# LanaSina/evolutionary_illusion_generator

Hardware: AMD Instinct MI355X
Metric: genome fitness evals/sec at 256x256, pop=256 (higher is better)
Workload: dtype f32; 1 GPU; neat_configs/circles.txt colour pop=256, 256x256, PredNet 3,48,96,192, 21 steps, LK + rotation-symmetry score; global_pop=256, genomes_per_gpu=256, device_batch=256, structure=Circles

## Files before the change

evolutionary_illusion_generator_amd/csrc/conv_wino4.h:

```cpp
#pragma once
#include "wino_launch.h"

namespace eig {

constexpr int W4_UPOS = 256;
constexpr int W4_U_FLOATS = W4_NPOS * W4_UPOS;
constexpr int W4_NUS = 3, W4_NPS = 3;
constexpr int w4_row(bool tall) { return tall ? 28 : 40; }
constexpr int w4_ps(bool tall) { return tall ? 1024 : 768; }
constexpr int w4_pslot(bool tall) { return W4_KC * w4_ps(tall); }
constexpr int w4_p(bool tall, int k) { return tall ? k * w4_pslot(true) : (k < 2 ? k * w4_pslot(false) : 2 * w4_pslot(false) + 3 * W4_U_FLOATS); }
constexpr int w4_u(bool tall, int k) { return tall ? 3 * w4_pslot(true) + k * W4_U_FLOATS : 2 * w4_pslot(false) + k * W4_U_FLOATS; }
constexpr int w4_x(bool tall) { return tall ? w4_u(true, 0) : w4_u(false, 1); }
constexpr int W4_X_FLOATS = W4_WAVES * 2 * 4 * 64 * 4;
constexpr int wino4_lds_bytes() { return (w4_x(false) + W4_X_FLOATS) * 4; }
static_assert((w4_u(true, 2) + W4_U_FLOATS) * 4 == wino4_lds_bytes() && (w4_p(false, 2) + w4_pslot(false)) * 4 <= wino4_lds_bytes(), "LDS maps");
#ifndef EIG_W4_DEEPU
#define EIG_W4_DEEPU 1
#endif
#ifndef EIG_W4_DIAG
#define EIG_W4_DIAG 0
#endif

__device__ __forceinline__ void w4_in1d(float d0, float d1, float d2, float d3, float d4, float d5, float* T)
{
    T[0] = fmaf(4.0f, d0, fmaf(-5.0f, d2, d4));
    const float p = fmaf(-4.0f, d2, d4), q = fmaf(-4.0f, d1, d3);
    T[1] = p + q; T[2] = p - q;
    const float r = d4 - d2, s = d3 - d1;
    T[3] = fmaf(2.0f, s, r); T[4] = fmaf(-2.0f, s, r);
    T[5] = fmaf(4.0f, d1, fmaf(-5.0f, d3, d5));
}
template <int XI> __device__ __forceinline__ float w4_row(const float* d)
{
    if constexpr (XI == 0) return fmaf(4.0f, d[0], fmaf(-5.0f, d[1], d[2]));
    else if constexpr (XI == 5) return fmaf(4.0f, d[0], fmaf(-5.0f, d[1], d[2]));
    else {
        if constexpr (XI == 1) return fmaf(-4.0f, d[1], d[3]) + fmaf(-4.0f, d[0], d[2]);
        else if constexpr (XI == 2) return fmaf(-4.0f, d[1], d[3]) - fmaf(-4.0f, d[0], d[2]);
        else if constexpr (XI == 3) return fmaf(2.0f, d[2] - d[0], d[3] - d[1]);
        else return fmaf(-2.0f, d[2] - d[0], d[3] - d[1]);
    }
}
constexpr int w4_nrows(int xi) { return (xi == 0 || xi == 5) ? 3 : 4; }
constexpr int w4_rowidx(int xi, int k) { return xi == 0 ? 2 * k : xi == 5 ? 2 * k + 1 : k + 1; }
constexpr int w4_uprow(int i) { return (i + 1) >> 1; }

template <typename V4> __device__ __forceinline__ void w4_out1d(const V4& m0, const V4& m1, const V4& m2, const V4& m3, const V4& m4, const V4& m5, V4* Y)
{
    const V4 s = m1 + m2, d = m1 - m2, u = m3 + m4, w = m3 - m4;
    Y[0] = (m0 + s) + u;
    for (int e = 0; e < 4; ++e) { Y[1][e] = fmaf(2.0f, w[e], d[e]); Y[2][e] = fmaf(4.0f, u[e], s[e]); Y[3][e] = fmaf(8.0f, w[e], d[e]) + m5[e]; }
}

template <int NI, int EPI, bool TALL = false, bool HALF = false, bool PACK = false, bool NSPLIT = false>
__global__ void __launch_bounds__((HALF && !NSPLIT) ? W4_THREADS / 2 : W4_THREADS, 3) wino4_kernel(const ConvArgs a)
{
    static_assert(!NSPLIT || (HALF && NI == 4 && EPI != EPI_CONVA), "N-split: a half block, 64-column N-blocks, ConvLSTM / ConvP");
    constexpr int NIW = NSPLIT ? 2 : NI;
    constexpr bool DEEPU = HALF && EIG_W4_DEEPU;
    static_assert(!(TALL && HALF), "half blocks exist in the wide shape only");
    static_assert(!PACK || (HALF && EPI != EPI_CONVA), "packed tiles: a half block, ConvLSTM / ConvP");
    constexpr bool TGEO = TALL || PACK;
    static_assert(EPI == EPI_LSTM || EPI == EPI_CONVA || EPI == EPI_CONVP, "conv_wino4.h: ConvLSTM, ConvA, ConvP");
    static_assert(EPI != EPI_LSTM || NI == 4, "ConvLSTM: the four N-tiles are the four gates");
    static_assert(NI == 3 || NI == 4, "N-blocks of 48 or 64 columns");
    constexpr int U4 = wino4_u_floats(NI);
    constexpr int KC = W4_KC, PS = w4_ps(TGEO), W4_ROW = w4_row(TGEO);
    constexpr int W4_P0 = w4_p(TGEO, 0), W4_P1 = w4_p(TGEO, 1), W4_P2 = w4_p(TGEO, 2), W4_U0 = w4_u(TGEO, 0), W4_U1 = w4_u(TGEO, 1), W4_U2 = w4_u(TGEO, 2);
    constexpr int PK_ROWS = 18, PK_CX = 7, PK_IMG = PK_ROWS * PK_CX;
    constexpr bool WALK = !TALL && !HALF;
    constexpr int RGH = TALL ? 16 : 8;
    extern __shared__ __attribute__((aligned(16))) float lds[];
    unsigned long long tq_entry = EIG_TIMING ? __builtin_readcyclecounter() : 0;
    float* const Pb = lds;
    float* const Ub = lds;
    float* const xb = lds + w4_x(TGEO);
    const int wv_o = __builtin_amdgcn_readfirstlane((int)threadIdx.x >> 6);
    const int rg_o = HALF ? 0 : wv_o & 1, xi_o = (HALF && !NSPLIT) ? wv_o : wv_o >> 1;
    const int ng_o = NSPLIT ? wv_o & 1 : 0;
    constexpr int NWAVES = (HALF && !NSPLIT) ? W4_WAVES / 2 : W4_WAVES;
    constexpr int UPW = 36 / NWAVES;
    auto lane_id = [&]() __attribute__((always_inline)) { int l = (int)__builtin_amdgcn_mbcnt_hi(~0u, __builtin_amdgcn_mbcnt_lo(~0u, 0u)); asm volatile("" : "+v"(l)); return l; };

    const int tiles = a.tilesX * a.tilesY;
    const bool pk5 = PACK && a.tilesX == 5;
    const int ntile = PACK ? a.B + (pk5 ? (a.B + 3) >> 2 : 0) : a.B * tiles;
    const int xcd = blockIdx.x & 7, xi_ = blockIdx.x >> 3;
    auto dv = [&](int x, int d, unsigned m) __attribute__((always_inline)) { return m ? (int)__umulhi((unsigned)x, m) : x / d; };
    const int q0 = dv(xi_, a.nparts, a.mg[0]);
    const int part = xi_ - q0 * a.nparts;
    const int tlin = a.tile_map ? xcd * ((ntile + 7) >> 3) + q0 : q0 * 8 + xcd;
    if (tlin >= ntile) return;
    const int nwalk = WALK ? a.nwalk : 1, nb0 = part * nwalk;
    const bool pk_edge_o = pk5 && tlin >= a.B;
    const int eb = PACK ? (pk_edge_o ? 4 * (tlin - a.B) : tlin) : dv(tlin, tiles, a.mg[1]);
    const int t_ = PACK ? 0 : tlin - eb * tiles;
    const int tyi = dv(t_, a.tilesX, a.mg[2]), txi = t_ - tyi * a.tilesX;
    const int y0 = PACK ? 0 : tyi * (TALL ? 32 : (HALF ? 8 : 16)), x0 = PACK ? 0 : txi * (TALL ? 16 : 32);
    const int HW = a.H * a.W;

    const bool up_fused = !PACK && EPI == EPI_LSTM && a.up_src != nullptr;
    const int nkb0 = a.src[0].C / KC;
    const int nkbu = up_fused ? (a.up_C / KC) : 0;
    const bool has1 = a.nsrc > 1;
    const int nkb_o = nkb0 + nkbu + (has1 ? (a.src[1].C / KC) : 0);
    const int up_lo_o = nkb0, up_hi_o = nkb0 + nkbu;
#define EIG4_WAITCNT(imm) do { __builtin_amdgcn_s_waitcnt(imm); asm volatile("" ::: "memory"); } while (0)
#define EIG4_BARRIER() do { asm volatile("" ::: "memory"); __builtin_amdgcn_s_barrier(); asm volatile("" ::: "memory"); } while (0)
#define EIG4_LDS_BARRIER() do { EIG4_WAITCNT(0xC07F); EIG4_BARRIER(); } while (0)
#define EIG4_IS_UP(kb) ((kb) >= up_lo && (kb) < up_hi)

    typedef float f32x2 __attribute__((ext_vector_type(2)));
    constexpr unsigned W4_POSB = 4 * 16 * NI * 4;
    auto walk_body = [&](const int it) __attribute__((always_inline)) {
    const int nblk = nb0 + it;
    int zs = 0;
    asm volatile("" : "+s"(zs));
    const int wv = wv_o + zs, rg = rg_o + zs, xi = xi_o + zs, ng = ng_o + zs, nkb = nkb_o + zs, up_lo = up_lo_o + zs, up_hi = up_hi_o + zs;
    const int pch = HALF ? wv >> 1 : wv / 3, ppart = HALF ? wv & 1 : wv - pch * 3;
    const bool has_plane = !(NSPLIT && !PACK) || wv_o < 8;
    const int eb_i = eb + zs, y0_i = y0 + zs, x0_i = x0 + zs;
    const bool pk_edge = (pk_edge_o ? 1 : 0) + zs != 0;
    const unsigned long long sb0 = (unsigned long long)(a.src[0].ptr + (size_t)eb_i * a.src[0].Ct * HW);
    const unsigned long long sb1 = has1 ? (unsigned long long)(a.src[1].ptr + (size_t)eb_i * a.src[1].Ct * HW) : sb0;
    const int ist0 = a.src[0].Ct * HW * 4, ist1 = has1 ? a.src[1].Ct * HW * 4 : ist0;
    const int sz0 = a.src[0].C * HW * 4 + (PACK ? 3 * ist0 : 0), sz1 = has1 ? a.src[1].C * HW * 4 + (PACK ? 3 * ist1 : 0) : sz0;
    const int Hh = a.H >> 1, Wh = a.W >> 1, HWh = Hh * Wh;
    const unsigned long long sbu = up_fused ? (unsigned long long)(a.up_src + (size_t)eb_i * a.up_C * HWh) : sb0;
    const int szu = up_fused ? a.up_C * HWh * 4 : sz0;
    const int lane = lane_id();
    const int q = lane >> 4, col = lane & 15;
    constexpr int CPR = TALL ? 7 : 10, CREAL = TALL ? 6 : 10, NCHK = TALL ? 34 * 7 : (HALF ? 100 : 180), UROWS = TALL ? 18 : (HALF ? 6 : 10), UCHK = TALL ? 4 : 6;
    auto plane_offsets = [&](int part, int& ro, int& uo) __attribute__((always_inline)) {
        const int c = lane + 64 * part;
        const int row = c / CPR, cx = c - row * CPR;
        const int gy = y0_i - 1 + row, gx = x0_i - 4 + 4 * cx;
        ro = (c < NCHK && cx < CREAL && gy >= 0 && gy < a.H && gx >= 0 && gx < a.W) ? (gy * a.W + gx) * 4 : -1;
        const int hy = (y0_i >> 1) - 1 + row, hx = (x0_i >> 1) - 4 + 4 * cx;
        uo = (row < UROWS && cx < UCHK && hy >= 0 && hy < Hh && hx >= 0 && hx < Wh) ? (hy * Wh + hx) * 4 : -1;
    };
    int pk_ro[3] = {-1, -1, -1};
    unsigned pk_mul[3] = {0u, 0u, 0u};
    const int pk_n = (wv_o < 4 ? 2 : 1) + (NSPLIT ? 0 : 1);
    if constexpr (PACK) {
#pragma unroll
        for (int k = 0; k < 3; ++k) {
            const int c = lane + 64 * ((wv_o + NWAVES * k) & 3);
            const int p = c >= PK_IMG ? 1 : 0, c1 = c - PK_IMG * p;
            const int row = c1 / PK_CX, slot = c1 - row * PK_CX;
            const int b = slot >= 3 ? (slot >= 6 ? 2 : 1) : 0;
            const int irel = pk_edge ? 2 * p + b : 0, cx = pk_edge ? 4 + slot - 3 * b : slot;
            const int gy = row - 1, gx = 4 * cx - 4;
            const bool ok = (pk_edge ? (c < 2 * PK_IMG && b < 2) : c < PK_IMG) && eb_i + irel < a.B && gy >= 0 && gy < a.H && gx >= 0 && gx < a.W;
            pk_ro[k] = ok ? (gy * a.W + gx) * 4 : -1;
            pk_mul[k] = ok ? (unsigned)irel : 0u;
        }
    }
    int roff, uoff, roff2 = -1, uoff2 = -1;
    plane_offsets(ppart, roff, uoff);
    const bool two_parts = (TALL && wv_o < 4) || (HALF && !PACK && !NSPLIT && wv_o < 2);
    if (TALL) plane_offsets(3, roff2, uoff2);
    if (HALF) { roff2 = roff; uoff2 = uoff; }
    const int ch2 = HALF ? 3 : wv, part2 = HALF ? ppart : 3;
    auto dma_plane_at = [&](int jj, int slot_off) __attribute__((always_inline)) {
        const int j = jj < nkb ? jj : nkb - 1;
        const bool up = EIG4_IS_UP(j);
        const bool s1 = j >= up_hi;
        const unsigned long long mu = 0ull - (unsigned long long)up, m1 = 0ull - (unsigned long long)s1;
        const unsigned long long u = sb0 + ((sb1 - sb0) & m1) + ((sbu - sb0) & mu);
        const unsigned lo = __builtin_amdgcn_readfirstlane((unsigned)u), hi = __builtin_amdgcn_readfirstlane((unsigned)(u >> 32));
        const int sz = sz0 + ((sz1 - sz0) & (int)m1) + ((szu - sz0) & (int)mu);
        const __amdgpu_buffer_rsrc_t rs = __builtin_amdgcn_make_buffer_rsrc((void*)(((unsigned long long)hi << 32) | lo), 0, __builtin_amdgcn_readfirstlane(sz), 0x00020000);
        const int base = (up_lo & (int)mu) + (up_hi & (int)m1), hw = HW + ((HWh - HW) & (int)mu);
        if constexpr (PACK) {
            const unsigned ist = (unsigned)(ist0 + ((ist1 - ist0) & (int)m1));
#pragma unroll
            for (int k = 0; k < 3; ++k) {
                if (k >= pk_n) break;
                const int idx = wv_o + NWAVES * k;
                const unsigned coffk = (unsigned)((j - base) * KC + (idx >> 2)) * (unsigned)(hw * 4);
                __builtin_amdgcn_raw_ptr_buffer_load_lds(rs, (__attribute__((address_space(3))) void*)(Pb + slot_off + (idx >> 2) * PS + (idx & 3) * 256), 16,
                                                         (int)__builtin_elementwise_add_sat((unsigned)pk_ro[k] + pk_mul[k] * ist, coffk), 0, 0, 0);
            }
            return;
        }
        if (!has_plane) return;
        const unsigned coff = (unsigned)((j - base) * KC + pch) * (unsigned)(hw * 4);
        __builtin_amdgcn_raw_ptr_buffer_load_lds(rs, (__attribute__((address_space(3))) void*)(Pb + slot_off + pch * PS + ppart * 256), 16,
                                                 (int)__builtin_elementwise_add_sat((unsigned)roff + (((unsigned)uoff - (unsigned)roff) & (unsigned)mu), coff), 0, 0, 0);
        if (two_parts) {
            const unsigned coff2 = (unsigned)((j - base) * KC + ch2) * (unsigned)(hw * 4);
            __builtin_amdgcn_raw_ptr_buffer_load_lds(rs, (__attribute__((address_space(3))) void*)(Pb + slot_off + ch2 * PS + part2 * 256), 16,
                                                     (int)__builtin_elementwise_add_sat((unsigned)roff2 + (((unsigned)uoff2 - (unsigned)roff2) & (unsigned)mu), coff2), 0, 0, 0);
        }
    };
    auto wait_u = [&]() __attribute__((always_inline)) {
        const int npl = PACK ? pk_n : (two_parts ? 2 : (has_plane ? 1 : 0));
        switch (npl + (DEEPU ? UPW : 0)) {
            case 0: EIG4_WAITCNT(0x0F70); break;
            case 1: EIG4_WAITCNT(0x0F71); break;
            case 2: EIG4_WAITCNT(0x0F72); break;
            case 3: EIG4_WAITCNT(0x0F73); break;
            case 4: EIG4_WAITCNT(0x0F74); break;
            case 5: EIG4_WAITCNT(0x0F75); break;
            case 6: EIG4_WAITCNT(0x0F76); break;
            case 7: EIG4_WAITCNT(0x0F77); break;
            case 8: EIG4_WAITCNT(0x0F78); break;
            default: EIG4_WAITCNT(0x0F79); break;
        }
    };
    const int uvo = (NI == 4 || lane < 48) ? lane * 16 : -1;
    auto prologue_a = [&](int nb) __attribute__((always_inline)) {
        const __amdgpu_buffer_rsrc_t rs = __builtin_amdgcn_make_buffer_rsrc((void*)(a.wpk + (size_t)nb * nkb * U4), 0, (nkb + 1) * U4 * 4, 0x00020000);
#pragma unroll
        for (int i = 0; i < UPW; ++i)
            __builtin_amdgcn_raw_ptr_buffer_load_lds(rs, (__attribute__((address_space(3))) void*)(Ub + W4_U0 + (UPW * wv + i) * W4_UPOS), 16, uvo, (int)((unsigned)(UPW * wv + i) * W4_POSB), 0, 0);
        dma_plane_at(0, W4_P0);
        dma_plane_at(1, W4_P1);
    };
    auto prologue_b = [&](int nb) __attribute__((always_inline)) {
        const __amdgpu_buffer_rsrc_t rs = __builtin_amdgcn_make_buffer_rsrc((void*)(a.wpk + (size_t)nb * nkb * U4), 0, (nkb + 1) * U4 * 4, 0x00020000);
#pragma unroll
        for (int i = 0; i < UPW; ++i)
            __builtin_amdgcn_raw_ptr_buffer_load_lds(rs, (__attribute__((address_space(3))) void*)(Ub + W4_U1 + (UPW * wv + i) * W4_UPOS), 16, uvo,
                                                     (int)((unsigned)U4 * 4 + (unsigned)(UPW * wv + i) * W4_POSB), 0, 0);
        dma_plane_at(2, W4_P2);
    };

    const int pk_ir = pk_edge ? col >> 2 : 0, pk_ty = pk_edge ? col & 3 : col >> 2;
    const int t_ty = PACK ? 0 : (TALL ? col >> 2 : col >> 3), t_tx = PACK ? (pk_edge ? 3 * (pk_ir & 1) : col & 3) : (TALL ? col & 3 : col & 7);
    const int pk_row = PACK ? PK_ROWS * (pk_ir >> 1) + 4 * pk_ty : 0;
    const float* const pbase_n = Pb + q * PS + (RGH * rg + 4 * t_ty + pk_row) * W4_ROW + 4 * t_tx;
    const float* const pbase_u = Pb + q * PS + ((RGH / 2) * rg + 2 * t_ty) * W4_ROW + 2 * t_tx + 3;
    const int b_off = xi * 6 * W4_UPOS + (q * 16 + col) * NI + 2 * ng;

    unsigned long long tq_setup = tq_entry;
    if (it == 0) {
        if (EIG_TIMING) tq_setup = __builtin_readcyclecounter();
        prologue_a(nb0);
        EIG4_WAITCNT(0x0F70);
    }
    const __amdgpu_buffer_rsrc_t rsw = __builtin_amdgcn_make_buffer_rsrc((void*)(a.wpk + (size_t)nblk * nkb * U4), 0, (nkb + 1) * U4 * 4, 0x00020000);
    unsigned u_so = (unsigned)(UPW * wv) * W4_POSB + 2u * (unsigned)U4 * 4u;
    auto dma_u = [&](int slot_off) __attribute__((always_inline)) {
#pragma unroll
        for (int i = 0; i < UPW; ++i)
            __builtin_amdgcn_raw_ptr_buffer_load_lds(rsw, (__attribute__((address_space(3))) void*)(Ub + slot_off + (UPW * wv + i) * W4_UPOS), 16, uvo,
                                                     (int)(u_so + (unsigned)i * W4_POSB), 0, 0);
        u_so += (unsigned)U4 * 4;
    };
    f32x4 acc[6][NIW];
#pragma unroll
    for (int p = 0; p < 6; ++p)
#pragma unroll
        for (int ni = 0; ni < NIW; ++ni) acc[p][ni] = (f32x4){0.f, 0.f, 0.f, 0.f};
    EIG4_BARRIER();
    prologue_b(nblk);
    const unsigned long long tq_k0 = EIG_TIMING ? __builtin_readcyclecounter() : 0;
    unsigned long long tq_k1 = 0, tq_x = 0, tq_y = 0;
    auto timeline = [&]() __attribute__((always_inline)) {
        if (EIG_TIMING && a.dbg && lane_id() == 0) {
            unsigned hwid, xcc;
            asm volatile("s_getreg_b32 %0, hwreg(HW_REG_HW_ID)" : "=s"(hwid));
            asm volatile("s_getreg_b32 %0, hwreg(HW_REG_XCC_ID)" : "=s"(xcc));
            unsigned long long* dd = a.dbg + (((size_t)blockIdx.x * nwalk + it) * NWAVES + wv) * 8;
            const unsigned long long tq_end = __builtin_readcyclecounter();
            dd[0] = tq_entry; dd[1] = tq_setup; dd[2] = tq_k0; dd[3] = tq_k1; dd[4] = tq_x; dd[5] = tq_y; dd[6] = tq_end;
            dd[7] = (unsigned long long)hwid | ((unsigned long long)xcc << 32);
            tq_entry = tq_end;
        }
    };

    auto kloops = [&](auto role_tag) __attribute__((always_inline)) {
        constexpr int XI = decltype(role_tag)::value;
        float v[6];
        float bq[NIW];
        int uo0 = W4_U0, uo1 = W4_U1, uo2 = W4_U2;
        int po0 = W4_P0, po1 = W4_P1, po2 = W4_P2;
        int pj = 0, psz = 0, pbound = 0;
        unsigned pcoff = 0, plo = 0, phi = 0, phw4 = 0, pist = 0;
        bool pup = false;
        auto plane_source = [&](int j) __attribute__((always_inline)) {
            const bool up = EIG4_IS_UP(j);
            const bool s1 = j >= up_hi;
            const unsigned long long mu = 0ull - (unsigned long long)up, m1 = 0ull - (unsigned long long)s1;
            const unsigned long long u = sb0 + ((sb1 - sb0) & m1) + ((sbu - sb0) & mu);
            plo = __builtin_amdgcn_readfirstlane((unsigned)u); phi = __builtin_amdgcn_readfirstlane((unsigned)(u >> 32));
            psz = __builtin_amdgcn_readfirstlane(sz0 + ((sz1 - sz0) & (int)m1) + ((szu - sz0) & (int)mu));
            const int base = (up_lo & (int)mu) + (up_hi & (int)m1);
            phw4 = (unsigned)((HW + ((HWh - HW) & (int)mu)) * 4);
            pcoff = (unsigned)((j - base) * KC + (PACK ? 0 : pch)) * phw4;
            if constexpr (PACK) pist = (unsigned)(ist0 + ((ist1 - ist0) & (int)m1));
            pup = up; pj = j;
            pbound = j < up_lo ? up_lo : (j < up_hi ? up_hi : nkb);
        };
        auto dma_plane = [&]() __attribute__((always_inline)) {
            const unsigned o = (unsigned)roff + (((unsigned)uoff - (unsigned)roff) & (0u - (unsigned)pup));
            const __amdgpu_buffer_rsrc_t prs = __builtin_amdgcn_make_buffer_rsrc((void*)(((unsigned long long)phi << 32) | plo), 0, psz, 0x00020000);
            if constexpr (PACK) {
#pragma unroll
                for (int k = 0; k < 3; ++k) {
                    if (k >= pk_n) break;
                    const int idx = wv + NWAVES * k;
                    __builtin_amdgcn_raw_ptr_buffer_load_lds(prs, (__attribute__((address_space(3))) void*)(Pb + po0 + (idx >> 2) * PS + (idx & 3) * 256), 16,
                                                             (int)__builtin_elementwise_add_sat((unsigned)pk_ro[k] + pk_mul[k] * pist, pcoff + (unsigned)(idx >> 2) * phw4), 0, 0, 0);
                }
            } else if (has_plane) {
            __builtin_amdgcn_raw_ptr_buffer_load_lds(prs, (__attribute__((address_space(3))) void*)(Pb + po0 + pch * PS + ppart * 256), 16,
                                                     (int)__builtin_elementwise_add_sat(o, pcoff), 0, 0, 0);
            }
            if (two_parts) {
                const unsigned o2 = (unsigned)roff2 + (((unsigned)uoff2 - (unsigned)roff2) & (0u - (unsigned)pup));
                __builtin_amdgcn_raw_ptr_buffer_load_lds(prs, (__attribute__((address_space(3))) void*)(Pb + po0 + ch2 * PS + part2 * 256), 16,
                                                         (int)__builtin_elementwise_add_sat(o2, pcoff + (unsigned)(ch2 - pch) * phw4), 0, 0, 0);
            }
            ++pj; pcoff += KC * phw4;
            if (__builtin_expect(pj == pbound, 0)) {
                if (pbound < nkb) plane_source(pj);
                else { --pj; pcoff -= KC * phw4; }
            }
        };
        plane_source(3 < nkb ? 3 : nkb - 1);
        float pr[2][6];
        float t[6];
        int rso = 0;
        bool rup = false;
        auto read_rows = [&](int ph) __attribute__((always_inline)) {
            if (EIG_W4_DIAG & 4) return;
            constexpr bool END = XI == 0 || XI == 5;
#pragma unroll
            for (int j = 0; j < 2; ++j) {
                const int k = ph == 0 ? (END ? 1 + j : 1 + 2 * j) : (END ? 0 : 2 * j);
                if (ph == 1 && END && j == 1) continue;
                if (rup) {
                    const float* const pl = pbase_u + rso + w4_uprow(w4_rowidx(XI, k)) * W4_ROW;
                    const float s0 = pl[0], s1_ = pl[1], s2 = pl[2], s3 = pl[3];
                    pr[j][0] = s0; pr[j][1] = s1_; pr[j][2] = s1_; pr[j][3] = s2; pr[j][4] = s2; pr[j][5] = s3;
                } else {
                    const float* const pl = pbase_n + rso + w4_rowidx(XI, k) * W4_ROW;
                    typedef const volatile __attribute__((address_space(3))) f32x2* lds_f32x2;
                    const f32x2 c0 = *(lds_f32x2)(pl + 2), c2 = *(lds_f32x2)(pl + 8);
                    const f32x4 c1 = *reinterpret_cast<const f32x4*>(pl + 4);
                    pr[j][0] = c0[1]; pr[j][1] = c1[0]; pr[j][2] = c1[1]; pr[j][3] = c1[2]; pr[j][4] = c1[3]; pr[j][5] = c2[0];
                }
            }
        };
        auto rows_begin = [&](int slot_off, bool up) __attribute__((always_inline)) {
            rso = slot_off; rup = up;
            read_rows(0);
        };
        auto rows_mid = [&]() __attribute__((always_inline)) {
            if (!(EIG_W4_DIAG & 4)) {
#pragma unroll
                for (int c = 0; c < 6; ++c) {
                    if constexpr (XI == 0 || XI == 5) t[c] = fmaf(-5.0f, pr[0][c], pr[1][c]);
                    else if constexpr (XI == 1 || XI == 2) t[c] = fmaf(-4.0f, pr[0][c], pr[1][c]);
                    else t[c] = pr[1][c] - pr[0][c];
                }
            }
            read_rows(1);
        };
        auto rows_end = [&]() __attribute__((always_inline)) {
            if (EIG_W4_DIAG & 4) return;
#pragma unroll
            for (int c = 0; c < 6; ++c) {
                if constexpr (XI == 0 || XI == 5) t[c] = fmaf(4.0f, pr[0][c], t[c]);
                else if constexpr (XI == 1) t[c] = t[c] + fmaf(-4.0f, pr[0][c], pr[1][c]);
                else if constexpr (XI == 2) t[c] = t[c] - fmaf(-4.0f, pr[0][c], pr[1][c]);
                else if constexpr (XI == 3) t[c] = fmaf(2.0f, pr[1][c] - pr[0][c], t[c]);
                else t[c] = fmaf(-2.0f, pr[1][c] - pr[0][c], t[c]);
            }
        };
        auto build_cols = [&]() __attribute__((always_inline)) {
            if (EIG_W4_DIAG & 4) { for (int c = 0; c < 6; ++c) v[c] = 1.0f; return; }
            w4_in1d(t[0], t[1], t[2], t[3], t[4], t[5], v);
        };
        auto read_b = [&](int slot_off, int nu, float* dst) __attribute__((always_inline)) {
            const float* const bsrc = Ub + slot_off + b_off + nu * W4_UPOS;
            if constexpr (NSPLIT) {
                const f32x2 b2 = *reinterpret_cast<const f32x2*>(bsrc);
                dst[0] = b2[0]; dst[1] = b2[1];
            } else if constexpr (NI == 4) {
                const f32x4 b4 = *reinterpret_cast<const f32x4*>(bsrc);
                dst[0] = b4[0]; dst[1] = b4[1]; dst[2] = b4[2]; dst[3] = b4[3];
            } else {
#pragma unroll
                for (int ni = 0; ni < NI; ++ni) dst[ni] = bsrc[ni];
            }
        };
        float bv[2][NIW];
        auto khead_mfma = [&]() __attribute__((always_inline)) {
            __builtin_amdgcn_sched_barrier(0);
            acc[0][0] = __builtin_amdgcn_mfma_f32_16x16x4f32(v[0], bq[0], acc[0][0], 0, 0, 0);
            __builtin_amdgcn_sched_barrier(0);
            read_b(uo0, 1, bv[1]);
#pragma unroll
            for (int ni = 1; ni < NIW; ++ni) acc[0][ni] = __builtin_amdgcn_mfma_f32_16x16x4f32(v[0], bq[ni], acc[0][ni], 0, 0, 0);
            __builtin_amdgcn_sched_barrier(0);
        };
        auto khead = [&](const int kb, auto kind_tag) __attribute__((always_inline)) {
            constexpr int KIND = decltype(kind_tag)::value;
            if constexpr (XI != 2 || KIND == 0) khead_mfma();
            else if constexpr (KIND == 2) khead_mfma();
        };
        auto ktail = [&](const int kb, auto kind_tag, auto nk_tag, auto last_tag, auto first_tag) __attribute__((always_inline)) {
            constexpr int KIND = decltype(kind_tag)::value;
            constexpr int NK = decltype(nk_tag)::value;
            constexpr bool LAST = decltype(last_tag)::value;
            constexpr bool FIRST = decltype(first_tag)::value || (DEEPU && !LAST);
            constexpr bool UP = KIND == 1;
            constexpr bool IDLE = UP && XI == 2;
            constexpr int NCH = IDLE ? 0 : (UP ? 5 : 6);
            auto slice = [&](int i) __attribute__((always_inline)) {
                if constexpr (!LAST) {
                    if (i == 0) { if (!(EIG_W4_DIAG & 16)) dma_u(uo2); }
                    if (i == 1) { if (!(EIG_W4_DIAG & 8)) dma_plane(); }
                    if (i == NCH - 4) rows_begin(po1, NK == 2 ? EIG4_IS_UP(kb + 1) : NK == 1);
                    if (i == NCH - 3) rows_mid();
                    if (i == NCH - 2) rows_end();
                    if (i == NCH - 1) build_cols();
                }
            };
            if constexpr (IDLE) {
                if constexpr (!LAST) {
                    if (!(EIG_W4_DIAG & 16)) dma_u(uo2);
                    if (!(EIG_W4_DIAG & 8)) dma_plane();
                    rows_begin(po1, NK == 2 ? EIG4_IS_UP(kb + 1) : NK == 1); rows_mid(); rows_end();
                    if constexpr (!FIRST) read_b(uo1, 0, bq);
                    build_cols();
                }
            } else {
                slice(0);
                __builtin_amdgcn_sched_barrier(0);
#pragma unroll
                for (int i = 1; i < NCH; ++i) {
                    const int nu = (UP && i >= 2) ? i + 1 : i;
                    if (i + 1 < NCH) {
                        const int nu1 = (UP && i + 1 >= 2) ? i + 2 : i + 1;
                        read_b(uo0, nu1, bv[(i + 1) & 1]);
                    } else if constexpr (!LAST && !FIRST) read_b(uo1, 0, bq);
                    const float* const b = bv[i & 1];
#pragma unroll
                    for (int ni = 0; ni < NIW; ++ni) acc[nu][ni] = __builtin_amdgcn_mfma_f32_16x16x4f32(v[nu], b[ni], acc[nu][ni], 0, 0, 0);
                    slice(i);
                    __builtin_amdgcn_sched_barrier(0);
                }
            }
            if constexpr (TALL && !LAST) asm volatile("" : "+v"(v[0]), "+v"(v[1]), "+v"(v[2]), "+v"(v[3]), "+v"(v[4]), "+v"(v[5]));
            { const int t0 = uo0; uo0 = uo1; uo1 = uo2; uo2 = t0; }
            { const int t0 = po0; po0 = po1; po1 = po2; po2 = t0; }
            if (LAST || (EIG_W4_DIAG & (8 | 16))) EIG4_WAITCNT(0x0F70);
            else if (!(EIG_W4_DIAG & 2)) { if (!(EIG_W4_DIAG & 1)) wait_u(); }
            if (!(EIG_W4_DIAG & 2) || LAST) EIG4_BARRIER();
            if constexpr (FIRST) read_b(uo0, 0, bq);
        };
        const std::false_type nl{};
        const std::integral_constant<int, 0> full{};
        const std::integral_constant<int, 2> rt{};
        int kb = 0;
        rows_begin(W4_P0, EIG4_IS_UP(0)); rows_mid(); rows_end();
        read_b(W4_U0, 0, bq);
        build_cols();
        EIG4_WAITCNT(0xC07F);
        EIG4_BARRIER();
        auto run = [&](const int end, auto kind_tag) __attribute__((always_inline)) {
            const int m = end - (end == nkb ? 1 : 0);
            for (; kb + 1 < m; ++kb) { ktail(kb, kind_tag, kind_tag, nl, nl); khead(kb + 1, kind_tag); }
            if (kb + 1 == m) { ktail(kb, kind_tag, rt, nl, nl); ++kb; khead(kb, rt); }
        };
        khead(0, full); ktail(0, full, full, nl, std::true_type{}); khead(1, full);
        kb = 1;
        run(up_lo, full);
        run(up_hi, std::integral_constant<int, 1>{});
        run(nkb, full);
        ktail(nkb - 1, rt, rt, std::true_type{}, nl);
    };
    switch (xi) {
        case 0: kloops(std::integral_constant<int, 0>{}); break;
        case 1: kloops(std::integral_constant<int, 1>{}); break;
        case 2: kloops(std::integral_constant<int, 2>{}); break;
        case 3: kloops(std::integral_constant<int, 3>{}); break;
        case 4: kloops(std::integral_constant<int, 4>{}); break;
        default: kloops(std::integral_constant<int, 5>{}); break;
    }
    if (EIG_TIMING) tq_k1 = __builtin_readcyclecounter();
    const bool more = it + 1 < nwalk;
    if (more) prologue_a(nblk + 1);

    f32x4 cc[4][NIW];
#pragma unroll
    for (int ni = 0; ni < NIW; ++ni) {
        f32x4 Y[4];
        w4_out1d(acc[0][ni], acc[1][ni], acc[2][ni], acc[3][ni], acc[4][ni], acc[5][ni], Y);
#pragma unroll
        for (int b = 0; b < 4; ++b) cc[b][ni] = Y[b];
    }
    {
    int zf = 0;
    asm volatile("" : "+s"(zf));
    const int eb = eb_i + zf, y0 = y0_i + zf, x0 = x0_i + zf, wv = wv_o + zf, rg = rg_o + zf, xi = xi_o + zf, HWf = HW + zf, Cout = a.Cout + zf, ngf = ng_o + zf;
    const bool pk_edge_f = (pk_edge_o ? 1 : 0) + zf != 0;
    const int lane = lane_id();
    const int q = lane >> 4, col = lane & 15;
    const size_t cHW = (size_t)HWf;
    const int j = TALL ? lane & 3 : lane & 7, chl = TALL ? lane >> 2 : lane >> 3, e_r = j & 3, ql = TALL ? 0 : j >> 2;
    int woff[4];
#pragma unroll
    for (int e = 0; e < 4; ++e) woff[e] = (((2 * xi + (NSPLIT ? ngf : rg)) * 2 * 4 + e) * 64 + q * 16 + ((col + 4 * e + (PACK ? q : (TALL ? 0 : 8 * (q & 1)))) & 15)) * 4;
    const int fr = lane & 15, fchl = lane >> 4;
    const int f_i = pk_edge_f ? fr >> 2 : 0, f_ty = pk_edge_f ? fr & 3 : fr >> 2, f_tx = pk_edge_f ? 4 : fr & 3;
    if constexpr (EPI == EPI_LSTM || EPI == EPI_CONVP) {
        const int nun = NSPLIT ? ((xi < 4 && ngf == 0) ? 2 : 1) : (xi < 4 ? 3 : 2);
        auto unit_cq = [&](int un) __attribute__((always_inline)) { return xi < 4 ? (NSPLIT ? (ngf ? 2 : un) : un) : 3; };
        auto unit_arow = [&](int un) __attribute__((always_inline)) { return xi < 4 ? xi : 2 * (xi - 4) + (NSPLIT ? ngf : un); };
        int xoff[3];
#pragma unroll
        for (int un = 0; un < 3; ++un) {
            const int cq = unit_cq(un);
            const int ty = TALL ? cq : cq >> 1, chh = TALL ? 0 : cq & 1;
            xoff[un] = TALL ? (e_r * 64 + ty * 16 + ((chl + 4 * e_r) & 15)) * 4 : (e_r * 64 + (2 * ty + ql) * 16 + ((8 * chh + chl + 4 * e_r + 8 * ql) & 15)) * 4;
            if constexpr (PACK) xoff[un] = ((fr & 3) * 64 + (fr >> 2) * 16 + ((4 * cq + fchl + 4 * (fr & 3) + (fr >> 2)) & 15)) * 4;
        }
        auto finish = [&](int arow, int nr, int off, int xw) __attribute__((always_inline)) -> f32x4 {
            auto C = [&](int x) __attribute__((always_inline)) { return *reinterpret_cast<const f32x4*>(xb + ((x * 2 + xw) * 2 + nr) * 1024 + off); };
            const f32x4 c1 = C(1), c2 = C(2), c3 = C(3), c4 = C(4);
            const f32x4 s_ = c1 + c2, d_ = c1 - c2, u_ = c3 + c4, w_ = c3 - c4;
            f32x4 y;
            if (arow == 0) { const f32x4 c0 = C(0); y = (c0 + s_) + u_; }
            else if (arow == 1) { for (int b = 0; b < 4; ++b) y[b] = fmaf(2.0f, w_[b], d_[b]); }
            else if (arow == 2) { for (int b = 0; b < 4; ++b) y[b] = fmaf(4.0f, u_[b], s_[b]); }
            else { const f32x4 c5 = C(5); for (int b = 0; b < 4; ++b) y[b] = fmaf(8.0f, w_[b], d_[b]) + c5[b]; }
            return y;
        };
        f32x4 ys[NI][3];
        auto finish_unit = [&](int ni, int nr, int xw, int un) __attribute__((always_inline)) {
            const int sel = NSPLIT ? ngf : un;
            switch (xi) {
                case 0: ys[ni][un] = finish(0, nr, xoff[un], xw); break;
                case 1: ys[ni][un] = finish(1, nr, xoff[un], xw); break;
                case 2: ys[ni][un] = finish(2, nr, xoff[un], xw); break;
                case 3: ys[ni][un] = finish(3, nr, xoff[un], xw); break;
                case 4: ys[ni][un] = sel ? finish(1, nr, xoff[un], xw) : finish(0, nr, xoff[un], xw); break;
                default: ys[ni][un] = sel ? finish(3, nr, xoff[un], xw) : finish(2, nr, xoff[un], xw); break;
            }
        };
        if constexpr (NSPLIT) {
#pragma unroll
            for (int nr = 0; nr < 2; ++nr)
#pragma unroll
                for (int e = 0; e < 4; ++e) {
                    f32x4 t;
                    t[0] = cc[0][nr][e]; t[1] = cc[1][nr][e]; t[2] = cc[2][nr][e]; t[3] = cc[3][nr][e];
                    *reinterpret_cast<f32x4*>(xb + woff[e] + nr * 1024) = t;
                }
            EIG4_LDS_BARRIER();
            if (EIG_TIMING) tq_x = __builtin_readcyclecounter();
#pragma unroll
            for (int ni = 0; ni < NI; ++ni)
#pragma unroll
                for (int un = 0; un < 2; ++un) {
                    if (un >= nun) break;
                    finish_unit(ni, ni & 1, ni >> 1, un);
                }
        } else {
#pragma unroll
        for (int rnd = 0; rnd < 2; ++rnd) {
            if (2 * rnd >= NI) break;
            if (rnd) EIG4_LDS_BARRIER();
#pragma unroll
            for (int nr = 0; nr < 2; ++nr) {
                const int ni = 2 * rnd + nr;
                if (ni >= NI) break;
#pragma unroll
                for (int e = 0; e < 4; ++e) {
                    f32x4 t;
                    t[0] = cc[0][ni][e]; t[1] = cc[1][ni][e]; t[2] = cc[2][ni][e]; t[3] = cc[3][ni][e];
                    *reinterpret_cast<f32x4*>(xb + woff[e] + nr * 1024) = t;
                }
            }
            EIG4_LDS_BARRIER();
            if (EIG_TIMING && rnd == 0) tq_x = __builtin_readcyclecounter();
#pragma unroll
            for (int nr = 0; nr < 2; ++nr) {
                const int ni = 2 * rnd + nr;
                if (ni >= NI) break;
#pragma unroll
                for (int un = 0; un < 3; ++un) {
                    if (un >= nun) break;
                    finish_unit(ni, nr, rg, un);
                }
            }
        }
        }
        if (more) EIG4_WAITCNT(0x0F70);
        if (EIG_TIMING) { asm volatile("s_waitcnt lgkmcnt(0)" ::: "memory"); tq_y = __builtin_readcyclecounter(); }
#pragma unroll
        for (int un = 0; un < 3; ++un) {
            if (un >= nun) break;
            const int cq = unit_cq(un);
            const int ty = TALL ? cq : cq >> 1, chh = TALL ? 0 : cq & 1;
            const int arow = unit_arow(un);
            const int gy = PACK ? 4 * f_ty + arow : y0 + RGH * rg + 4 * ty + arow, gx = PACK ? 4 * f_tx : x0 + 4 * j;
            if (gy >= a.H || gx >= a.W) continue;
            const int ebo = PACK ? eb + f_i : eb;
            if (PACK && ebo >= a.B) continue;
            const size_t pix = (size_t)gy * a.W + gx;
            const int chq = PACK ? 4 * cq + fchl : 8 * chh + chl;
            if constexpr (EPI == EPI_LSTM) {
                const int ch = nblk * 16 + chq;
                if (ch >= Cout) continue;
                const float bi = a.bias[ch], bf = a.bias[Cout + ch], bc = a.bias[2 * Cout + ch], bo = a.bias[3 * Cout + ch];
                const size_t cbase = ((size_t)ebo * Cout + ch) * cHW, ps = (size_t)Cout * cHW, pbase = (size_t)ch * cHW;
                const f32x4 cold4 = *reinterpret_cast<const f32x4*>(a.c_state + cbase + pix);
                const f32x4 pi4 = *reinterpret_cast<const f32x4*>(a.peep + pbase + pix);
                const f32x4 pf4 = *reinterpret_cast<const f32x4*>(a.peep + ps + pbase + pix);
                const f32x4 po4 = *reinterpret_cast<const f32x4*>(a.peep + 2 * ps + pbase + pix);
                f32x4 cn4, hn4;
#pragma unroll
                for (int b = 0; b < 4; ++b) {
                    float cn, hn;
                    lstm_cell(ys[0][un][b], ys[1][un][b], ys[2][un][b], ys[3][un][b], bi, bf, bc, bo, cold4[b], pi4[b], pf4[b], po4[b], cn, hn);
                    cn4[b] = cn; hn4[b] = hn;
                }
                *reinterpret_cast<f32x4*>(a.c_state + cbase + pix) = cn4;
                *reinterpret_cast<f32x4*>(a.h_out + cbase + pix) = hn4;
            } else {
#pragma unroll
                for (int ni = 0; ni < NI; ++ni) {
                    const int ch = (nblk * NI + ni) * 16 + chq;
                    if (ch >= Cout) continue;
                    const float bb_ = a.bias[ch];
                    f32x4 v4;
#pragma unroll
                    for (int b = 0; b < 4; ++b) v4[b] = relu_f(ys[ni][un][b] + bb_);
                    *reinterpret_cast<f32x4*>(a.Pout + ((size_t)ebo * Cout + ch) * cHW + pix) = v4;
                }
            }
        }
    } else {
        const int Ho = a.H >> 1, Wo = a.W >> 1;
        const size_t plane = (size_t)Ho * Wo;
        const int ox = (x0 >> 1) + 2 * j;
#pragma unroll
        for (int rnd = 0; rnd < 2; ++rnd) {
            if (2 * rnd >= NI) break;
            const int nval = NI - 2 * rnd >= 2 ? 2 : 1;
            if (rnd) EIG4_LDS_BARRIER();
#pragma unroll
            for (int nr = 0; nr < 2; ++nr) {
                if (nr >= nval) break;
                const int ni = 2 * rnd + nr;
#pragma unroll
                for (int e = 0; e < 4; ++e) {
                    f32x4 t;
                    t[0] = cc[0][ni][e]; t[1] = cc[1][ni][e]; t[2] = cc[2][ni][e]; t[3] = cc[3][ni][e];
                    *reinterpret_cast<f32x4*>(xb + woff[e] + nr * 1024) = t;
                }
            }
            EIG4_LDS_BARRIER();
            if (rnd == (NI - 1) / 2) { if (more) EIG4_WAITCNT(0x0F70); }
            if (EIG_TIMING && rnd == 0) { tq_x = __builtin_readcyclecounter(); tq_y = tq_x; }
            const int g0 = nval == 2 ? (xi < 4 ? 3 * xi : 12 + 2 * (xi - 4)) : (xi < 2 ? 2 * xi : xi + 2);
            const int cnt = nval == 2 ? (xi < 4 ? 3 : 2) : (xi < 2 ? 2 : 1);
#pragma unroll
            for (int un = 0; un < 3; ++un) {
                if (un >= cnt) break;
                const int g = g0 + un;
                const int nr = g >> 3, ty = TALL ? (g >> 1) & 3 : (g >> 2) & 1, ap = TALL ? g & 1 : (g >> 1) & 1, chh = TALL ? 0 : g & 1;
                const int off = TALL ? ((nr + 2 * rg) * 256 + e_r * 64 + ty * 16 + ((chl + 4 * e_r) & 15)) * 4
                                     : ((nr + 2 * rg) * 256 + e_r * 64 + (2 * ty + ql) * 16 + ((8 * chh + chl + 4 * e_r + 8 * ql) & 15)) * 4;
                auto C = [&](int x) __attribute__((always_inline)) { return *reinterpret_cast<const f32x4*>(xb + x * 4096 + off); };
                const f32x4 c1 = C(1), c2 = C(2), c3 = C(3), c4 = C(4);
                const f32x4 s_ = c1 + c2, d_ = c1 - c2, u_ = c3 + c4, w_ = c3 - c4;
                f32x4 ya, yb;
                if (ap == 0) {
                    const f32x4 c0 = C(0);
                    ya = (c0 + s_) + u_;
                    for (int b = 0; b < 4; ++b) yb[b] = fmaf(2.0f, w_[b], d_[b]);
                } else {
                    const f32x4 c5 = C(5);
                    for (int b = 0; b < 4; ++b) { ya[b] = fmaf(4.0f, u_[b], s_[b]); yb[b] = fmaf(8.0f, w_[b], d_[b]) + c5[b]; }
                }
                const int ch = (nblk * NI + 2 * rnd + nr) * 16 + 8 * chh + chl;
                const int oy = (y0 >> 1) + (RGH / 2) * rg + 2 * ty + ap;
                if (oy >= Ho || ox >= Wo || ch >= Cout) continue;
                const float bb_ = a.bias[ch];
                const size_t pb = ((size_t)eb * Cout + ch) * plane + (size_t)oy * Wo + ox;
                const size_t e0 = ((size_t)eb * 2 * Cout + ch) * plane + (size_t)oy * Wo + ox, e1 = e0 + (size_t)Cout * plane;
                const f32x2 p2 = *reinterpret_cast<const f32x2*>(a.P + pb);
                f32x2 ea, eb2;
#pragma unroll
                for (int bp = 0; bp < 2; ++bp) {
                    const float v00 = relu_f(ya[2 * bp] + bb_), v01 = relu_f(ya[2 * bp + 1] + bb_);
                    const float v10 = relu_f(yb[2 * bp] + bb_), v11 = relu_f(yb[2 * bp + 1] + bb_);
                    const float A = fmaxf(fmaxf(v00, v01), fmaxf(v10, v11));
                    ea[bp] = relu_f(A - p2[bp]);
                    eb2[bp] = relu_f(p2[bp] - A);
                }
                *reinterpret_cast<f32x2*>(a.E + e0) = ea;
                *reinterpret_cast<f32x2*>(a.E + e1) = eb2;
            }
        }
    }
    }
    timeline();
    };
    for (int it = 0; it < nwalk; ++it) walk_body(it);
#undef EIG4_WAITCNT
#undef EIG4_BARRIER
#undef EIG4_LDS_BARRIER
#undef EIG4_IS_UP
}

}
```

evolutionary_illusion_generator_amd/csrc/weight_pack.h:

```cpp
#pragma once
#include <cmath>
#include <cstddef>
#include <vector>

#include "wino_geom.h"

namespace eig {

inline int pad4(int c) { return (c + 3) & ~3; }

struct PackGeom {
    int NI = 4, n_nblk = 0, krows = 0, Cout = 0;
    int nsrc = 0;
    int src_C[3] = {0, 0, 0};
    int src_Ct[3] = {0, 0, 0};
};

inline std::vector<float> pack_weights(const PackGeom& op, const float* const srcw[3][4], int lstm)
{
    const int NB = op.NI * 16;
    std::vector<float> out((size_t)op.n_nblk * op.krows * NB, 0.0f);
    for (int nb = 0; nb < op.n_nblk; ++nb) {
        size_t row = 0;
        for (int s = 0; s < op.nsrc; ++s) {
            const int Cin = op.src_C[s], Cp = pad4(Cin);
            const int Cw = op.src_Ct[s] ? op.src_Ct[s] : Cin;
            for (int c = 0; c < Cp; ++c)
                for (int tap = 0; tap < 9; ++tap, ++row) {
                    if (c >= Cin) continue;
                    float* dst = &out[((size_t)nb * op.krows + row) * NB];
                    for (int n = 0; n < NB; ++n) {
                        int g = 0, o;
                        if (lstm == 1) { g = n / 16; o = nb * 16 + (n % 16); }
                        else if (lstm == 2) { g = n / 4; o = n % 4; }
                        else o = nb * NB + n;
                        if (o >= op.Cout) continue;
                        dst[(n % 16) * op.NI + (n / 16)] = srcw[s][g][((size_t)o * Cw + c) * 9 + tap];
                    }
                }
        }
    }
    return out;
}

inline float presum_up_weight(const float* w9, int py, int px, int a, int b)
{
    const int ky0 = py ? (a ? 2 : 0) : (a ? 1 : 0), ky1 = py ? (a ? 2 : 1) : (a ? 2 : 0);
    const int kx0 = px ? (b ? 2 : 0) : (b ? 1 : 0), kx1 = px ? (b ? 2 : 1) : (b ? 2 : 0);
    volatile float s = 0.0f;
    bool first = true;
    for (int ky = ky0; ky <= ky1; ++ky)
        for (int kx = kx0; kx <= kx1; ++kx) {
            if (first) { s = w9[ky * 3 + kx]; first = false; }
            else s = s + w9[ky * 3 + kx];
        }
    return s;
}

inline std::vector<float> pack_weights_up4(const PackGeom& op, const float* const srcw[4], int lstm)
{
    const int NB = op.NI * 16;
    const int Cin = op.src_C[0];
    std::vector<float> out((size_t)4 * op.n_nblk * op.krows * NB, 0.0f);
    for (int cls = 0; cls < 4; ++cls)
        for (int nb = 0; nb < op.n_nblk; ++nb)
            for (int c = 0; c < Cin; ++c)
                for (int tap = 0; tap < 4; ++tap) {
                    float* dst = &out[(((size_t)cls * op.n_nblk + nb) * op.krows + (size_t)c * 4 + tap) * NB];
                    for (int n = 0; n < NB; ++n) {
                        int g = 0, o;
                        if (lstm == 1) { g = n / 16; o = nb * 16 + (n % 16); }
                        else if (lstm == 2) { g = n / 4; o = n % 4; }
                        else o = nb * NB + n;
                        if (o >= op.Cout) continue;
                        dst[(n % 16) * op.NI + (n / 16)] = presum_up_weight(srcw[g] + ((size_t)o * Cin + c) * 9, cls >> 1, cls & 1, tap >> 1, tap & 1);
                    }
                }
    return out;
}

inline std::vector<float> pack_weights_up4c(const PackGeom& op, const float* const srcw[4], int lstm)
{
    const int Cin = op.src_C[0];
    std::vector<float> out((size_t)op.n_nblk * op.krows * 64, 0.0f);
    for (int nb = 0; nb < op.n_nblk; ++nb)
        for (int c = 0; c < Cin; ++c)
            for (int tap = 0; tap < 4; ++tap)
                for (int n = 0; n < 16; ++n) {
                    int g = 0, o;
                    if (lstm == 2) { g = n / 4; o = n % 4; }
                    else o = nb * 16 + n;
                    if (o >= op.Cout) continue;
                    for (int cls = 0; cls < 4; ++cls)
                        out[(((size_t)nb * op.krows + (size_t)c * 4 + tap) * 16 + n) * 4 + cls] =
                            presum_up_weight(srcw[g] + ((size_t)o * Cin + c) * 9, cls >> 1, cls & 1, tap >> 1, tap & 1);
                }
    return out;
}

inline void wino4_w1d(float g0, float g1, float g2, float* W)
{
    const float c6 = -1.0f / 6.0f, c24 = 1.0f / 24.0f;
    W[0] = 0.25f * g0;
    const float a = g0 + g2;
    W[1] = (a + g1) * c6; W[2] = (a - g1) * c6;
    const float b = fmaf(4.0f, g2, g0);
    W[3] = fmaf(2.0f, g1, b) * c24; W[4] = fmaf(-2.0f, g1, b) * c24;
    W[5] = g2;
}
inline void wino4_weight(const float* g, float* U)
{
    float s[6][3], W[6];
    for (int j = 0; j < 3; ++j) { wino4_w1d(g[j], g[3 + j], g[6 + j], W); for (int i = 0; i < 6; ++i) s[i][j] = W[i]; }
    for (int i = 0; i < 6; ++i) wino4_w1d(s[i][0], s[i][1], s[i][2], U + i * 6);
}
inline std::vector<float> pack_weights_wino(int C, int NI, int n_nblk, bool lstm, int nsrc, const int* src_C, const int* src_Cw, const float* const srcw[3][4])
{
    const int kc = W4_KC;
    int nkb = 0;
    for (int s = 0; s < nsrc; ++s) nkb += src_C[s] / kc;
    const int npos = W4_NPOS;
    const int uf = wino4_u_floats(NI);
    std::vector<float> out((size_t)n_nblk * nkb * uf + uf, 0.0f);
    float U[36];
    for (int nb = 0; nb < n_nblk; ++nb) {
        int kb0 = 0;
        for (int s = 0; s < nsrc; ++s) {
            for (int c = 0; c < src_C[s]; ++c)
                for (int ni = 0; ni < NI; ++ni)
                    for (int n = 0; n < 16; ++n) {
                        const int o = lstm ? nb * 16 + n : (nb * NI + ni) * 16 + n;
                        if (o >= C) continue;
                        wino4_weight(srcw[s][lstm ? ni : 0] + ((size_t)o * src_Cw[s] + c) * 9, U);
                        float* dst = &out[((size_t)nb * nkb + kb0 + c / kc) * uf];
                        for (int pos = 0; pos < npos; ++pos) dst[((pos * kc + (c % kc)) * 16 + n) * NI + ni] = U[pos];
                    }
            kb0 += src_C[s] / kc;
        }
    }
    return out;
}

inline std::vector<float> lstm0_raw_table(int C, const float* const wx0[4], const float* const wh[4])
{
    const int K = 3 * C * 9, K0 = C * 9;
    std::vector<float> raw((size_t)C * K * 4 + (size_t)C * K0 * 4);
    for (int o = 0; o < C; ++o)
        for (int g = 0; g < 4; ++g) {
            for (int c = 0; c < 2 * C; ++c)
                for (int t9 = 0; t9 < 9; ++t9) {
                    const float wv = wx0[g][((size_t)o * 2 * C + c) * 9 + t9];
                    raw[((size_t)o * K + c * 9 + t9) * 4 + g] = wv;
                    if (c < C) raw[(size_t)C * K * 4 + ((size_t)o * K0 + c * 9 + t9) * 4 + g] = wv;
                }
            for (int c = 0; c < C; ++c)
                for (int t9 = 0; t9 < 9; ++t9) raw[((size_t)o * K + (2 * C + c) * 9 + t9) * 4 + g] = wh[g][((size_t)o * C + c) * 9 + t9];
        }
    return raw;
}

}
```

evolutionary_illusion_generator_amd/csrc/wino_geom.h:

```cpp
#pragma once

namespace eig {

constexpr int W4_WAVES = 12;
constexpr int W4_THREADS = 64 * W4_WAVES;
constexpr int W4_KC = 4;
constexpr int W4_NPOS = 36;
constexpr int wino4_u_floats(int NI) { return W4_NPOS * 4 * 16 * NI; }

enum { W4_WIDE = 0, W4_TALL = 1, W4_HALF = 2, W4_PACK = 3 };

}
```

Measured before the change: 441.8 genome evals/s.

## Pad Winograd weight layout to four outputs and reschedule B reads and column build

Pads the packed Winograd weight tile so each output position always holds four entries, even when only three are used. This lets the NI=3 path use single 16-byte LDS vector reads and full-wave DMA instead of scalar reads with lane masking. It also precomputes LDS base pointers, reads the second B fragment early for NI=3, and moves build_cols one slice earlier for non-LSTM epilogues to overlap with the MFMAs. The cost is more weight memory and DMA traffic for NI=3 and higher register pressure.

```diff
diff --git a/evolutionary_illusion_generator_amd/csrc/conv_wino4.h b/evolutionary_illusion_generator_amd/csrc/conv_wino4.h
--- a/evolutionary_illusion_generator_amd/csrc/conv_wino4.h
+++ b/evolutionary_illusion_generator_amd/csrc/conv_wino4.h
@@ -3,7 +3,7 @@
 
 namespace eig {
 
-constexpr int W4_UPOS = 256;
+constexpr int W4_UPOS = 4 * 16 * W4_NIP;
 constexpr int W4_U_FLOATS = W4_NPOS * W4_UPOS;
 constexpr int W4_NUS = 3, W4_NPS = 3;
 constexpr int w4_row(bool tall) { return tall ? 28 : 40; }
@@ -112,7 +112,7 @@
 #define EIG4_IS_UP(kb) ((kb) >= up_lo && (kb) < up_hi)
 
     typedef float f32x2 __attribute__((ext_vector_type(2)));
-    constexpr unsigned W4_POSB = 4 * 16 * NI * 4;
+    constexpr unsigned W4_POSB = W4_UPOS * 4;
     auto walk_body = [&](const int it) __attribute__((always_inline)) {
     const int nblk = nb0 + it;
     int zs = 0;
@@ -210,7 +210,7 @@
             default: EIG4_WAITCNT(0x0F79); break;
         }
     };
-    const int uvo = (NI == 4 || lane < 48) ? lane * 16 : -1;
+    const int uvo = lane * 16;
     auto prologue_a = [&](int nb) __attribute__((always_inline)) {
         const __amdgpu_buffer_rsrc_t rs = __builtin_amdgcn_make_buffer_rsrc((void*)(a.wpk + (size_t)nb * nkb * U4), 0, (nkb + 1) * U4 * 4, 0x00020000);
 #pragma unroll
@@ -233,7 +233,7 @@
     const int pk_row = PACK ? PK_ROWS * (pk_ir >> 1) + 4 * pk_ty : 0;
     const float* const pbase_n = Pb + q * PS + (RGH * rg + 4 * t_ty + pk_row) * W4_ROW + 4 * t_tx;
     const float* const pbase_u = Pb + q * PS + ((RGH / 2) * rg + 2 * t_ty) * W4_ROW + 2 * t_tx + 3;
-    const int b_off = xi * 6 * W4_UPOS + (q * 16 + col) * NI + 2 * ng;
+    const int b_off = xi * 6 * W4_UPOS + (q * 16 + col) * W4_NIP + 2 * ng;
 
     unsigned long long tq_setup = tq_entry;
     if (it == 0) {
@@ -276,6 +276,8 @@
         constexpr int XI = decltype(role_tag)::value;
         float v[6];
         float bq[NIW];
+        constexpr bool B1_EARLY = NI == 3;
+        float bq1[NIW];
         int uo0 = W4_U0, uo1 = W4_U1, uo2 = W4_U2;
         int po0 = W4_P0, po1 = W4_P1, po2 = W4_P2;
         int pj = 0, psz = 0, pbound = 0;
@@ -376,25 +378,31 @@
             if (EIG_W4_DIAG & 4) { for (int c = 0; c < 6; ++c) v[c] = 1.0f; return; }
             w4_in1d(t[0], t[1], t[2], t[3], t[4], t[5], v);
         };
-        auto read_b = [&](int slot_off, int nu, float* dst) __attribute__((always_inline)) {
-            const float* const bsrc = Ub + slot_off + b_off + nu * W4_UPOS;
+        typedef const __attribute__((address_space(3))) float* lds_cf;
+        auto read_b = [&](lds_cf ub, int nu, float* dst) __attribute__((always_inline)) {
+            const float* const bsrc = (const float*)(ub + nu * W4_UPOS);
             if constexpr (NSPLIT) {
                 const f32x2 b2 = *reinterpret_cast<const f32x2*>(bsrc);
                 dst[0] = b2[0]; dst[1] = b2[1];
-            } else if constexpr (NI == 4) {
+            } else {
                 const f32x4 b4 = *reinterpret_cast<const f32x4*>(bsrc);
-                dst[0] = b4[0]; dst[1] = b4[1]; dst[2] = b4[2]; dst[3] = b4[3];
-            } else {
-#pragma unroll
-                for (int ni = 0; ni < NI; ++ni) dst[ni] = bsrc[ni];
+#pragma unroll
+                for (int ni = 0; ni < NI; ++ni) dst[ni] = b4[ni];
             }
         };
         float bv[2][NIW];
+        lds_cf ubc = (lds_cf)(Ub + W4_U0 + b_off), ubn = ubc;
+        auto ub_cur = [&]() __attribute__((always_inline)) { return TALL ? (lds_cf)(Ub + uo0 + b_off) : ubc; };
+        auto ub_next = [&]() __attribute__((always_inline)) { return TALL ? (lds_cf)(Ub + uo1 + b_off) : ubn; };
+        auto read_bq = [&](lds_cf ub) __attribute__((always_inline)) {
+            read_b(ub, 0, bq);
+            if constexpr (B1_EARLY) read_b(ub, 1, bq1);
+        };
         auto khead_mfma = [&]() __attribute__((always_inline)) {
             __builtin_amdgcn_sched_barrier(0);
             acc[0][0] = __builtin_amdgcn_mfma_f32_16x16x4f32(v[0], bq[0], acc[0][0], 0, 0, 0);
             __builtin_amdgcn_sched_barrier(0);
-            read_b(uo0, 1, bv[1]);
+            if constexpr (!B1_EARLY) read_b(ub_cur(), 1, bv[1]);
 #pragma unroll
             for (int ni = 1; ni < NIW; ++ni) acc[0][ni] = __builtin_amdgcn_mfma_f32_16x16x4f32(v[0], bq[ni], acc[0][ni], 0, 0, 0);
             __builtin_amdgcn_sched_barrier(0);
@@ -412,14 +420,17 @@
             constexpr bool UP = KIND == 1;
             constexpr bool IDLE = UP && XI == 2;
             constexpr int NCH = IDLE ? 0 : (UP ? 5 : 6);
+            constexpr bool COLS_EARLY = EPI != EPI_LSTM;
+            float vl = 0.0f;
+            auto next_ub = [&]() __attribute__((always_inline)) { if constexpr (!TALL) { ubn = ubc + (uo1 - uo0); asm volatile("" : "+v"(ubn)); } };
             auto slice = [&](int i) __attribute__((always_inline)) {
                 if constexpr (!LAST) {
                     if (i == 0) { if (!(EIG_W4_DIAG & 16)) dma_u(uo2); }
                     if (i == 1) { if (!(EIG_W4_DIAG & 8)) dma_plane(); }
                     if (i == NCH - 4) rows_begin(po1, NK == 2 ? EIG4_IS_UP(kb + 1) : NK == 1);
                     if (i == NCH - 3) rows_mid();
-                    if (i == NCH - 2) rows_end();
-                    if (i == NCH - 1) build_cols();
+                    if (i == NCH - 2) { rows_end(); next_ub(); if (COLS_EARLY) build_cols(); }
+                    if (i == NCH - 1 && !COLS_EARLY) build_cols();
                 }
             };
             if constexpr (IDLE) {
@@ -427,7 +438,8 @@
                     if (!(EIG_W4_DIAG & 16)) dma_u(uo2);
                     if (!(EIG_W4_DIAG & 8)) dma_plane();
                     rows_begin(po1, NK == 2 ? EIG4_IS_UP(kb + 1) : NK == 1); rows_mid(); rows_end();
-                    if constexpr (!FIRST) read_b(uo1, 0, bq);
+                    next_ub();
+                    if constexpr (!FIRST) read_bq(ub_next());
                     build_cols();
                 }
             } else {
@@ -438,11 +450,14 @@
                     const int nu = (UP && i >= 2) ? i + 1 : i;
                     if (i + 1 < NCH) {
                         const int nu1 = (UP && i + 1 >= 2) ? i + 2 : i + 1;
-                        read_b(uo0, nu1, bv[(i + 1) & 1]);
-                    } else if constexpr (!LAST && !FIRST) read_b(uo1, 0, bq);
-                    const float* const b = bv[i & 1];
-#pragma unroll
-                    for (int ni = 0; ni < NIW; ++ni) acc[nu][ni] = __builtin_amdgcn_mfma_f32_16x16x4f32(v[nu], b[ni], acc[nu][ni], 0, 0, 0);
+                        read_b(ub_cur(), nu1, bv[(i + 1) & 1]);
+                    } else if constexpr (!LAST && !FIRST) read_bq(ub_next());
+                    const float* const b = (B1_EARLY && i == 1) ? bq1 : bv[i & 1];
+                    const float va = (COLS_EARLY && !LAST && i == NCH - 1) ? vl : v[nu];
+#pragma unroll
+                    for (int ni = 0; ni < NIW; ++ni) acc[nu][ni] = __builtin_amdgcn_mfma_f32_16x16x4f32(va, b[ni], acc[nu][ni], 0, 0, 0);
+                    __builtin_amdgcn_sched_barrier(0);
+                    if (COLS_EARLY && !LAST && i == NCH - 2) vl = v[5];
                     slice(i);
                     __builtin_amdgcn_sched_barrier(0);
                 }
@@ -450,17 +465,18 @@
             if constexpr (TALL && !LAST) asm volatile("" : "+v"(v[0]), "+v"(v[1]), "+v"(v[2]), "+v"(v[3]), "+v"(v[4]), "+v"(v[5]));
             { const int t0 = uo0; uo0 = uo1; uo1 = uo2; uo2 = t0; }
             { const int t0 = po0; po0 = po1; po1 = po2; po2 = t0; }
+            ubc = ubn;
             if (LAST || (EIG_W4_DIAG & (8 | 16))) EIG4_WAITCNT(0x0F70);
             else if (!(EIG_W4_DIAG & 2)) { if (!(EIG_W4_DIAG & 1)) wait_u(); }
             if (!(EIG_W4_DIAG & 2) || LAST) EIG4_BARRIER();
-            if constexpr (FIRST) read_b(uo0, 0, bq);
+            if constexpr (FIRST) read_bq(ub_cur());
         };
         const std::false_type nl{};
         const std::integral_constant<int, 0> full{};
         const std::integral_constant<int, 2> rt{};
         int kb = 0;
         rows_begin(W4_P0, EIG4_IS_UP(0)); rows_mid(); rows_end();
-        read_b(W4_U0, 0, bq);
+        read_bq(ub_cur());
         build_cols();
         EIG4_WAITCNT(0xC07F);
         EIG4_BARRIER();
diff --git a/evolutionary_illusion_generator_amd/csrc/weight_pack.h b/evolutionary_illusion_generator_amd/csrc/weight_pack.h
--- a/evolutionary_illusion_generator_amd/csrc/weight_pack.h
+++ b/evolutionary_illusion_generator_amd/csrc/weight_pack.h
@@ -133,7 +133,7 @@
                         if (o >= C) continue;
                         wino4_weight(srcw[s][lstm ? ni : 0] + ((size_t)o * src_Cw[s] + c) * 9, U);
                         float* dst = &out[((size_t)nb * nkb + kb0 + c / kc) * uf];
-                        for (int pos = 0; pos < npos; ++pos) dst[((pos * kc + (c % kc)) * 16 + n) * NI + ni] = U[pos];
+                        for (int pos = 0; pos < npos; ++pos) dst[((pos * kc + (c % kc)) * 16 + n) * W4_NIP + ni] = U[pos];
                     }
             kb0 += src_C[s] / kc;
         }
diff --git a/evolutionary_illusion_generator_amd/csrc/wino_geom.h b/evolutionary_illusion_generator_amd/csrc/wino_geom.h
--- a/evolutionary_illusion_generator_amd/csrc/wino_geom.h
+++ b/evolutionary_illusion_generator_amd/csrc/wino_geom.h
@@ -6,7 +6,8 @@
 constexpr int W4_THREADS = 64 * W4_WAVES;
 constexpr int W4_KC = 4;
 constexpr int W4_NPOS = 36;
-constexpr int wino4_u_floats(int NI) { return W4_NPOS * 4 * 16 * NI; }
+constexpr int W4_NIP = 4;
+constexpr int wino4_u_floats(int ) { return W4_NPOS * 4 * 16 * W4_NIP; }
 
 enum { W4_WIDE = 0, W4_TALL = 1, W4_HALF = 2, W4_PACK = 3 };
 
```

After: 439.2 genome evals/s. No clear change (-0.6%).
